# abdel-habib/mmg-clip

Measured on AMD Instinct MI355X. Metric: image-text pairs/sec (global batch), higher is better.
Workload: dtype bf16; 1 GPU; C2: train_binary_class_clf, ConvNeXt-tiny 1024x1024x1 + BERT-base S=77, LinearProjection 768->512, CLIPLoss, AdamW, all parameters trained; global_batch=256, per_gpu_batch=256, micro_batch=256, streams=text tower on a side stream, parallelism=dp1, loss_scope=local, text_dropout=HF training-mode dropout live (hidden 0.1, atte…

## Files before the change

include/mmgclip_hip.h:

```cpp
#ifndef MMGCLIP_HIP_H
#define MMGCLIP_HIP_H

#ifdef __cplusplus
extern "C" {
#endif

typedef void* mmg_stream_t;

int mmg_abi_version(void);
const char* mmg_last_error(void);
const char* mmg_target_arch(void);
int mmg_device_cu_count(void);
int mmg_set_kernel_notes(int on);
const char* mmg_last_kernel(void);
const char* mmg_gemm_plan(int op, int M, int N, int K, int cus);


int mmg_l2norm_fwd(const float* x, float* y, float* norm, int rows, int D, mmg_stream_t stream);
int mmg_l2norm_bwd(const float* y, const float* norm, const float* dy, float* dx, int rows, int D,
                   mmg_stream_t stream);

int mmg_clip_rows_fwd(const float* X, const float* Y, const float* scale, int n_loc, int N, int D, int diag_off,
                      float* lse, float* pos, float* logits, int ldl, mmg_stream_t stream);

// ... 31 lines not shown
int mmg_layernorm_bwd_f32(const void* dy, int lddy, const float* x, int ldx, const float* mean, const float* rstd,
                          const float* gamma, void* dx, int lddx, float* dgamma, float* dbeta, int M, int C,
                          const void* add, int ldadd, mmg_stream_t stream);
int mmg_layernorm_bwd(const void* dy, int lddy, const void* x, int ldx, const float* mean, const float* rstd,
                      const float* gamma, void* dx, int lddx, float* dgamma, float* dbeta, int M, int C, int patch,
                      int H, int W, const void* add, int ldadd, mmg_stream_t stream);
const char* mmg_layernorm_plan(int door, int M, int C, int res, int yf, int add);

int mmg_gelu_fwd_bf16(const void* x, void* y, long long n, mmg_stream_t stream);
int mmg_act_grad_bf16(const void* dy, const void* pre, void* out, long long n, int kind, mmg_stream_t stream);
int mmg_cast_f32_bf16(const float* x, void* y, long long n, mmg_stream_t stream);
int mmg_cast_bf16_f32(const void* x, float* y, long long n, mmg_stream_t stream);
int mmg_transpose_cast_bf16(const float* src, int R, int C, const float* rowscale, void* dst, int ldd,
                            mmg_stream_t stream);

int mmg_avgpool_fwd(const void* x, float* y, int n, int HW, int C, mmg_stream_t stream);
int mmg_avgpool_bwd(const float* dy, void* dx, int n, int HW, int C, mmg_stream_t stream);

int mmg_view_pool_fwd(const float* feat, const int* offsets, float* out, int* argmax, int S, int C, int mode, mmg_stream_t stream);
int mmg_view_pool_bwd(const float* dout, const int* offsets, const int* argmax, float* dfeat, int S, int V, int C, int mode,
                      mmg_stream_t stream);

int mmg_patchify(const float* img, void* out, int n, int Cin, int H, int W, int P, int Kp, int scale16,
                 mmg_stream_t stream);
int mmg_patchify_aug(const void* img, int src_kind, void* out, int n, int Cin, int H, int W, int P, int Kp, int scale16,
                     const int* geom, const float* tone, mmg_stream_t stream);

int mmg_adamw_step(float* p, const float* g, float* m, float* v, void* p_bf16, long long n, float lr, float beta1,
                   float beta2, float eps, float weight_decay, int step, float grad_scale, mmg_stream_t stream);


int mmg_grad_sumsq_partials(long long n);
int mmg_grad_sumsq(const float* g, long long n, double* partials, int n_partials, mmg_stream_t stream);
int mmg_grad_clip_finalize(const double* partials, int n, float max_norm, float* out, int* skipped, mmg_stream_t stream);
int mmg_adamw_step_guarded(float* p, const float* g, float* m, float* v, void* p_bf16, long long n, float lr, float beta1,
                           float beta2, float eps, float weight_decay, int step, const float* clip, const int* skipped,
                           mmg_stream_t stream);
int mmg_adamw_step_groups(float* p, const float* g, float* m, float* v, long long n, const unsigned char* chunk_group, int n_groups,
                          const float* group_lr, const float* group_wd, float beta1, float beta2, float eps, int step,
                          const float* clip, const int* skipped, mmg_stream_t stream);

int mmg_layerscale_finalize(const float* W2, const float* b2, const float* gamma, const float* dW2raw,
                            const float* db2raw, float* dW2, float* db2, float* dgamma, int C, int K,
                            mmg_stream_t stream);
int mmg_grad_relayout(const float* src, float* dst, int mode, int R, int CI, int KH, int KW, int ld_src,
                      mmg_stream_t stream);

int mmg_image_swap(void* x, const int* pairs, const int* pairs_host, int k, int n, long long rows, int C, mmg_stream_t stream);
int mmg_image_copy(const void* src, void* dst, int first, int count, int n, long long rows, int C, mmg_stream_t stream);
int mmg_scaled_add_f32(float* dst, const float* src, float alpha, long long n, mmg_stream_t stream);

int mmg_dropout_fwd(const float* x, float* y, void* keep, long long n, float p, long long seed, mmg_stream_t stream);
int mmg_dropout_bwd(const float* dy, const void* keep, float* dx, long long n, float p, mmg_stream_t stream);


int mmg_dwconv7_nhwc(const void* x, const float* w, const float* bias, const void* add, void* y, int n, int H, int W,
                     int C, int flip, mmg_stream_t stream);
int mmg_dwconv7_nhwc_mfma(const void* x, const float* w, const float* bias, const void* add, void* y, int n, int H, int W,
                          int C, int flip, mmg_stream_t stream);
int mmg_dwconv7_wgrad(const void* x, const void* dy, float* dw, float* dbias, int n, int H, int W, int C,
                      mmg_stream_t stream);


long long mmg_cnblock_packed_elems(int C, int backward);
int mmg_cnblock_pack_weights(const float* w1, const float* w2, const float* gamma, void* packed, int C, int backward,
                             mmg_stream_t stream);
int mmg_cnblock_mlp_fwd(const void* xd, const float* ln_w, const float* ln_b, float eps, const void* packed,
                        const float* b1, const float* b2, const float* gamma, const void* residual, void* y, void* hpre,
                        void* xln, void* gact, float* mean, float* rstd, int hpre_kind, long long M, int C, mmg_stream_t stream);

int mmg_cnblock_mlp_bwd_supported(int C);
int mmg_cnblock_mlp_bwd(const void* dy, const void* xd, const float* ln_w, const float* ln_b, float eps,
                        const void* packed_bwd, const float* b1, const void* hpre, void* dh, void* g, void* xln,
                        void* dxln, float* mean, float* rstd, float* ln_dw, float* ln_db, long long M, int C,
                        mmg_stream_t stream);

int mmg_cnblock_bwdw_supported(int C);
long long mmg_cnblock_bwdw_packed_elems(int C);
int mmg_cnblock_bwdw_pack(const float* w1, const float* w2, const float* ln_w, const float* ln_b, const float* layer_scale,
                          const float* b1, void* packed, float* b1f, int C, mmg_stream_t stream);
int mmg_cnblock_bwdw(const void* dy, const void* xd, const float* ln_w, const float* ln_b, float eps, const void* packed,
                     const float* b1f, void* dd, float* dW1, float* db1, float* dW2raw, float* db2raw, float* ln_dw,
                     float* ln_db, long long M, int C, mmg_stream_t stream);


int mmg_greedy_threshold_labels(const float* sim, int ld, int n, float threshold, long long* labels, int* counts, int* k_out,
                                mmg_stream_t stream);

int mmg_cluster_mean_cols_fwd(const float* logits, int ld, int n, int N, const long long* labels, const int* counts, int k,
                              float* out, int ldo, mmg_stream_t stream);
int mmg_cluster_mean_cols_bwd(const float* dout, int ldo, int n, int N, const long long* labels, const int* counts,
                              float* dlogits, int ld, mmg_stream_t stream);

int mmg_clip_labelled_rows_fwd(const float* X, const float* Y, const float* scale, const long long* row_label, int n_loc, int M,
                               int D, float* lse, float* pos, mmg_stream_t stream);
int mmg_clip_labelled_rows_bwd_row(const float* X, const float* Y, const float* scale, const float* lse_row,
                                   const long long* row_label, const float* gout, float coef, int n_loc, int M, int D,
                                   int accumulate, float* dX, float* dscale, mmg_stream_t stream);
int mmg_clip_labelled_rows_bwd_col(const float* X, const float* Y, const float* scale, const float* lse_col,
                                   const long long* col_label, const long long* row_key, int key_off, const int* counts,
                                   int n_counts, const float* gout, float coef, int n_loc, int M, int D, int accumulate,
                                   float* dX, mmg_stream_t stream);
int mmg_cluster_centroids(const float* T, const long long* labels, int N, int D, int k, float* out, mmg_stream_t stream);


int mmg_gemm_nt_fp8(const void* A, int lda, const void* B, int ldb, void* C, int ldc, int M, int N, int K,
                    const float* bias, const float* colscale, const void* residual, int ldr, void* aux_out, int ldao,
                    int epi, int out_kind, float alpha, const float* alpha_dev, mmg_stream_t stream);


int mmg_quantize_e5m2_bf16(const void* src, long long n, float* amax, void* dst, float* scales, mmg_stream_t stream);
int mmg_quantize_e5m2_bf16_delayed(const void* src, long long n, const float* amax_prev, float* amax_next, void* dst, float* scales,
                                   mmg_stream_t stream);
int mmg_quantize_e5m2_colsum_bf16(const void* src, int M, int C, const float* amax_prev, float* amax_next, void* dst, float* scales,
                                  float* colsum, mmg_stream_t stream);
int mmg_gemm_nt_fp8_bwd(const void* A, int lda, int a_e5m2, const void* B, int ldb, void* C, int ldc, int M, int N, int K,
                        const void* aux_in, int ldai, int epi, int out_kind, float alpha, const float* alpha_dev,
                        const float* alpha_dev2, mmg_stream_t stream);
int mmg_gemm_tn_fp8(const void* A, int lda, int a_e5m2, const void* B, int ldb, float* C, int ldc, int M, int N1, int N2,
                    float alpha, const float* alpha_dev, float* colsum_a, mmg_stream_t stream);

int mmg_absmax_f32(const float* src, long long n, float* amax, mmg_stream_t stream);
int mmg_quantize_e4m3_f32(const float* src, long long n, const float* amax, void* dst, float* scales, mmg_stream_t stream);

int mmg_layernorm_fwd_fp8(const void* x, int ldx, const float* gamma, const float* beta, float eps, void* y8, int ldy,
                          float* mean, float* rstd, int M, int C, mmg_stream_t stream);


int mmg_im2col_nhwc(const void* x, void* col, int n, int H, int W, int C, int KH, int KW, int stride, int pad, int Kp,
                    mmg_stream_t stream);
int mmg_col2im_nhwc(const void* dcol, void* dx, int n, int H, int W, int C, int KH, int KW, int stride, int pad, int Kp,
                    mmg_stream_t stream);
int mmg_maxpool3x3s2_nhwc(const void* x, void* y, int n, int H, int W, int C, mmg_stream_t stream);
int mmg_bn_stats_f64(const void* x, int M, int C, double* sum, double* sumsq, mmg_stream_t stream);
int mmg_bn_finalize_f64(const double* sum, const double* sumsq, int M, int C, const float* gamma, const float* beta, float eps,
                        float momentum, float* running_mean, float* running_var, int train, float* mean, float* rstd,
                        float* scale, float* shift, mmg_stream_t stream);
int mmg_bn_apply(const void* x, const float* scale, const float* shift, const void* residual, void* y, int M, int C, int relu,
                 mmg_stream_t stream);
int mmg_bn_bwd_reduce(const void* dy, const void* x, const void* out, const float* mean, const float* rstd, int M, int C,
                      float* sum_g, float* sum_gx, mmg_stream_t stream);
int mmg_bn_bwd_apply(const void* dy, const void* x, const void* out, const float* mean, const float* rstd, const float* gamma,
                     const float* sum_g, const float* sum_gx, int M, int C, void* dx, void* dres, float* dgamma, float* dbeta,
                     mmg_stream_t stream);


int mmg_attention_fwd(const void* qkv, int ld, const long long* mask, void* ctx, int ldc, float* lse, int B, int S,
                      int heads, int Hd, float scale, mmg_stream_t stream);
int mmg_attention_bwd(const void* qkv, int ld, const long long* mask, const void* ctx, int ldc, const float* lse,
                      const void* dctx, int lddc, void* dqkv, int lddq, int B, int S, int heads, int Hd, float scale,
                      mmg_stream_t stream);

int mmg_attention_long_fwd(const void* qkv, int ld, const long long* mask, void* ctx, int ldc, float* lse, int B, int S,
                           int heads, int Hd, float scale, mmg_stream_t stream);
int mmg_attention_long_bwd(const void* qkv, int ld, const long long* mask, const void* ctx, int ldc, const float* lse,
                           const void* dctx, int lddc, void* dqkv, int lddq, float* delta_ws, int B, int S, int heads,
                           int Hd, float scale, mmg_stream_t stream);

int mmg_attention_varlen_fwd(const void* qkv, int ld, const int* cu_seqlens, void* ctx, int ldc, float* lse, int B, int S_max,
                             int heads, int Hd, float scale, mmg_stream_t stream);
int mmg_attention_varlen_bwd(const void* qkv, int ld, const int* cu_seqlens, const void* ctx, int ldc, const float* lse,
                             const void* dctx, int lddc, void* dqkv, int lddq, int B, int S_max, int heads, int Hd,
                             float scale, mmg_stream_t stream);

int mmg_attention_dropout_fwd(const void* qkv, int ld, const long long* mask, const int* cu_seqlens, void* ctx, int ldc,
                              float* lse, int B, int S, int heads, int Hd, float scale, float p, unsigned long long seed,
// ... 35 lines not shown
```

mmg-clip_amd/mmgclip/kernels.py:

```python
import ctypes
import os

import torch

from . import _hip
from ._hip import call, ptr, stream
from .profile import PROFILE

BF16 = torch.bfloat16


def layernorm_fwd(x, gamma, beta, eps, patch_hw=None, want_stats=True):
    M, C = x.shape
    if patch_hw is None:
        y = torch.empty(M, C, device=x.device, dtype=BF16)
        patch, H, W = 0, 0, 0
    else:
        H, W = patch_hw
        y = torch.empty((M // (H * W)) * (H // 2) * (W // 2), 4 * C, device=x.device, dtype=BF16)
        patch = 1
    mean = torch.empty(M, device=x.device, dtype=torch.float32) if want_stats else None
    rstd = torch.empty(M, device=x.device, dtype=torch.float32) if want_stats else None
    PROFILE.timed("layernorm_fwd_kernel", 8.0 * M * C, 4 * M * C,
                  lambda: call("mmg_layernorm_fwd", ptr(x), x.stride(0), ptr(gamma), ptr(beta), float(eps), ptr(y), y.stride(0), ptr(mean),
# ... 117 lines not shown

def avgpool_bwd(dy, n, HW, C, out=None):
    dx = out if out is not None else torch.empty(n * HW, C, device=dy.device, dtype=BF16)
    call("mmg_avgpool_bwd", ptr(dy), ptr(dx), n, HW, C, stream())
    return dx


def _images(x, n):
    assert x.dtype == BF16 and x.dim() == 2 and x.is_contiguous() and n > 0 and x.shape[0] % n == 0, "bf16 [n * rows, C], contiguous"
    _hip.require_gpu(x)
    return x.shape[0] // n, x.shape[1]


def image_swap_(x, n, pairs_dev, pairs_host, k, offset=0):
    rows, C = _images(x, n)
    if k:
        assert pairs_dev.dtype == torch.int32 and pairs_dev.is_contiguous() and 2 * (offset + k) <= pairs_dev.numel() == len(pairs_host)
    call("mmg_image_swap", ptr(x), ctypes.c_void_p(pairs_dev.data_ptr() + 8 * offset) if k else None,
         ctypes.c_void_p(ctypes.addressof(pairs_host) + 8 * offset) if k else None, k, n, rows, C, stream())
    return x


def image_copy(src, dst, n, first, count):
    rows, C = _images(src, n)
    assert dst.shape == src.shape and dst.dtype == BF16 and dst.is_contiguous()
    _hip.require_gpu(dst)
    call("mmg_image_copy", ptr(src), ptr(dst), first, count, n, rows, C, stream())
    return dst


def scaled_add_(dst, src, alpha):
    assert dst.dtype == src.dtype == torch.float32 and dst.is_contiguous() and src.is_contiguous() and dst.numel() == src.numel()
    _hip.require_gpu(dst, src)
    call("mmg_scaled_add_f32", ptr(dst), ptr(src), float(alpha), dst.numel(), stream())
    return dst


def view_pool_fwd(feat, offsets, S, mode, out=None, argmax=None):
    V, C = feat.shape
    assert feat.dtype == torch.float32 and feat.is_contiguous() and offsets.dtype == torch.int32 and offsets.numel() == S + 1
    _hip.require_gpu(feat, offsets)
    y = out if out is not None else torch.empty(S, C, device=feat.device, dtype=torch.float32)
    if mode == 1 and argmax is None:
        argmax = torch.empty(S, C, device=feat.device, dtype=torch.int32)
    call("mmg_view_pool_fwd", ptr(feat), ptr(offsets), ptr(y), ptr(argmax) if mode == 1 else None, S, C, mode, stream())
    return y, (argmax if mode == 1 else None)


def view_pool_bwd(dout, offsets, argmax, V, mode, out=None):
    S, C = dout.shape
    assert dout.dtype == torch.float32 and dout.is_contiguous() and offsets.dtype == torch.int32 and offsets.numel() == S + 1
    _hip.require_gpu(dout, offsets)
    dx = out if out is not None else torch.empty(V, C, device=dout.device, dtype=torch.float32)
    call("mmg_view_pool_bwd", ptr(dout), ptr(offsets), ptr(argmax), ptr(dx), S, V, C, mode, stream())
    return dx


PIXEL_KINDS = {torch.float32: 0, torch.uint16: 1, torch.uint8: 2}


def stack_images(images):
    if images[0].dtype == torch.uint16:
        return torch.stack([t.view(torch.int16) for t in images]).view(torch.uint16)
    return torch.stack(list(images))


def patchify(img, P, Kp, scale16, geom=None, tone=None):
    n, Cin, H, W = img.shape
    if img.dtype not in PIXEL_KINDS:
        raise TypeError(f"pixels must be float32 in [0, 1], uint16 or uint8, got {img.dtype}")
    assert img.is_contiguous(), "pixels must be contiguous [n, Cin, H, W]"
    _hip.require_gpu(img, geom, tone)
    out = torch.empty(n * (H // P) * (W // P), Kp, device=img.device, dtype=BF16)
    if img.dtype == torch.float32 and geom is None and tone is None:
        call("mmg_patchify", ptr(img), ptr(out), n, Cin, H, W, P, Kp, 1 if scale16 else 0, stream())
        return out
    assert geom is None or (geom.dtype == torch.int32 and geom.is_contiguous() and tuple(geom.shape) == (n, 4)), "geom: int32 [n, 4]"
    assert tone is None or (tone.dtype == torch.float32 and tone.is_contiguous() and tuple(tone.shape) == (n, 2)), "tone: fp32 [n, 2]"
    call("mmg_patchify_aug", ptr(img), PIXEL_KINDS[img.dtype], ptr(out), n, Cin, H, W, P, Kp, 1 if scale16 else 0, ptr(geom), ptr(tone),
         stream())
    return out


def adamw_step(p, g, m, v, p16, lr, beta1, beta2, eps, wd, step, grad_scale=1.0):
    call("mmg_adamw_step", ptr(p), ptr(g), ptr(m), ptr(v), ptr(p16), p.numel(), float(lr), float(beta1), float(beta2),
         float(eps), float(wd), int(step), float(grad_scale), stream())


def grad_sumsq_partials(n):
    return int(_hip.load().mmg_grad_sumsq_partials(int(n)))


def grad_sumsq(g, partials, offset=0, count=None):
    assert g.dtype == torch.float32 and g.is_contiguous() and partials.dtype == torch.float64 and partials.is_contiguous()
    _hip.require_gpu(g, partials)
    count = grad_sumsq_partials(g.numel()) if count is None else int(count)
    assert 0 <= offset and offset + count <= partials.numel()
    call("mmg_grad_sumsq", ptr(g), g.numel(), ptr(partials[offset:]) if count else ptr(partials), count, stream())


def grad_clip_finalize(partials, n, max_norm, out, skipped=None):
    assert partials.dtype == torch.float64 and out.dtype == torch.float32 and out.numel() >= 3 and n <= partials.numel()
    assert skipped is None or (skipped.dtype == torch.int32 and skipped.numel() >= 1)
    _hip.require_gpu(partials, out, skipped)
    call("mmg_grad_clip_finalize", ptr(partials), int(n), 0.0 if max_norm is None else float(max_norm), ptr(out), ptr(skipped), stream())


def adamw_step_guarded(p, g, m, v, p16, lr, beta1, beta2, eps, wd, step, clip, skipped=None):
    assert clip.dtype == torch.float32 and clip.numel() >= 3 and (skipped is None or skipped.dtype == torch.int32)
    call("mmg_adamw_step_guarded", ptr(p), ptr(g), ptr(m), ptr(v), ptr(p16), p.numel(), float(lr), float(beta1), float(beta2),
         float(eps), float(wd), int(step), ptr(clip), ptr(skipped), stream())


ADAMW_MAX_GROUPS = 128


def adamw_step_groups(p, g, m, v, chunk_group, group_lr, group_wd, beta1, beta2, eps, step, clip=None, skipped=None):
    n_groups = len(group_lr)
    assert len(group_wd) == n_groups and chunk_group.dtype == torch.uint8 and chunk_group.is_contiguous()
    assert chunk_group.numel() * 64 == p.numel() == g.numel() == m.numel() == v.numel()
    assert clip is None or (clip.dtype == torch.float32 and clip.numel() >= 3)
    assert skipped is None or skipped.dtype == torch.int32
    _hip.require_gpu(p, g, m, v, chunk_group, clip, skipped)
    lrs = (ctypes.c_float * max(n_groups, 1))(*[float(x) for x in group_lr])
    wds = (ctypes.c_float * max(n_groups, 1))(*[float(x) for x in group_wd])
    call("mmg_adamw_step_groups", ptr(p), ptr(g), ptr(m), ptr(v), p.numel(), ptr(chunk_group), n_groups, lrs, wds, float(beta1),
         float(beta2), float(eps), int(step), ptr(clip), ptr(skipped), stream())


def dwconv_mfma_pays(n, H, W, C, flip):
    return H * W >= 96 * 96 and C <= 256


def dwconv7(x, w49, bias, n, H, W, C, add=None, flip=False, out=None):
    y = out if out is not None else torch.empty(n * H * W, C, device=x.device, dtype=BF16)
    px = n * H * W * C
    mode = os.environ.get("MMG_DWCONV_MFMA", "auto")
    if mode == "1" or (mode == "auto" and dwconv_mfma_pays(n, H, W, C, flip)):
        PROFILE.timed("dwconv7_mfma_kernel", 98.0 * px, (6 if add is not None else 4) * px,
                      lambda: call("mmg_dwconv7_nhwc_mfma", ptr(x), ptr(w49), ptr(bias), ptr(add), ptr(y), n, H, W, C, 1 if flip else 0, stream()),
                      f"n={n} {H}x{W} C={C}" + (" +add" if add is not None else ""))
        return y
    fam = "dwconv7_rows2_kernel" if os.environ.get("MMG_DWCONV_ROWS2", "1") != "0" else "dwconv7_kernel"
    PROFILE.timed(fam, 98.0 * px, (6 if add is not None else 4) * px,
                  lambda: call("mmg_dwconv7_nhwc", ptr(x), ptr(w49), ptr(bias), ptr(add), ptr(y), n, H, W, C, 1 if flip else 0, stream()),
                  f"n={n} {H}x{W} C={C}" + (" +add" if add is not None else ""))
    return y


def dwconv7_wgrad(x, dy, dw49, dbias, n, H, W, C):
    px = n * H * W * C
    fam = "dwconv7_wgrad_rows2_kernel" if os.environ.get("MMG_DWCONV_ROWS2", "1") != "0" else "dwconv7_wgrad_kernel"
    PROFILE.timed(fam, 98.0 * px, 4 * px,
                  lambda: call("mmg_dwconv7_wgrad", ptr(x), ptr(dy), ptr(dw49), ptr(dbias), n, H, W, C, stream()), f"n={n} {H}x{W} C={C}")


def cnblock_supported(C):
    return C in (96, 128, 192, 256, 384, 512)


def cnblock_pack(w1, w2, gamma=None, backward=False):
    C = w1.shape[1]
    backward = int(backward)
    n = _hip.load().mmg_cnblock_packed_elems(C, backward)
    if n <= 0:
        raise ValueError(f"fused CNBlock MLP: C={C} is not supported")
# ... 225 lines not shown
```

mmg-clip_amd/mmgclip/networks/convnext.py:

```python
import ctypes
import os

import torch
import torch.nn as nn

from .. import _hip
from .. import kernels as K
from .. import linalg as L
from .._hip import call, ptr, stream
from ..params import backward_finished, last_backward
from . import convnext_sd as SD
from .convnext_plan import BlockSaved, Knobs, decide_saves, fused_forward, plan_block, saving_form
from .tower import Tower, as_pixels, augment_tables, backward_parts, conv_weight_rows, fold_conv_grad, forward_parts

CONFIGS = {
    "tiny": dict(depths=(3, 3, 9, 3), dims=(96, 192, 384, 768)),
    "small": dict(depths=(3, 3, 27, 3), dims=(96, 192, 384, 768)),
    "base": dict(depths=(3, 3, 27, 3), dims=(128, 256, 512, 1024)),
}
LN_EPS = 1e-6


def _fused_save_maxc():
    return int(os.environ.get("MMG_MLP_FUSED_SAVE_MAXC", "384"))
# ... 110 lines not shown
                w1, w2, gamma = blk.block[3].weight.data, blk.block[5].weight.data, blk.layer_scale.data.reshape(C)
                if scales is not None and scales[b] != 1.0:
                    gamma = gamma * scales[b]
                wc[key + ".gamma"] = gamma
                b += 1
                wc[key + ".w49"] = blk.block[0].weight.data.reshape(C, 49).t().contiguous()
                wc[key + ".w1"] = K.cast_bf16(w1)
                wc[key + ".w1t"] = K.transpose_cast_bf16(w1)
                wc[key + ".w2"] = K.cast_bf16(w2)
                wc[key + ".w2gt"] = K.transpose_cast_bf16(w2, gamma)
                if p.kind == "fp8":
                    wc[key + ".w1f8"], wc[key + ".s1"] = K.quantize_e4m3(w1)
                    wc[key + ".w2f8"], wc[key + ".s2"] = K.quantize_e4m3(w2)
                    if p.fp8_bwd_weights:
                        wc[key + ".w2gt8"], wc[key + ".s2gt"] = K.quantize_e4m3((w2 * gamma.reshape(C, 1)).t().contiguous())
                        wc[key + ".w1t8"], wc[key + ".s1t"] = K.quantize_e4m3(w1.t().contiguous())
                elif p.kind == "fused":
                    wc[key + ".mlp"] = K.cnblock_pack(w1, w2)
                    if p.fused_bwd:
                        wc[key + ".mlpb"] = K.cnblock_pack(w1, w2, gamma, backward=p.fused_bwd)
                    if p.bwdw:
                        wc[key + ".bwdw"] = K.cnblock_bwdw_pack(w1, w2, blk.block[2].weight.data, blk.block[2].bias.data, gamma,
                                                                blk.block[3].bias.data)
            if si < 3:
                wds = conv_weight_rows(f[2 + 2 * si][1].weight.data)
                wc[f"ds{si}.w"] = K.cast_bf16(wds)
                wc[f"ds{si}.wt"] = K.transpose_cast_bf16(wds)
        return wc

    def _decide_saves(self, n_alive, H, W, device, ckpt=False, more=()):
        return decide_saves(self.plan or self._plan_blocks(), self.depths, ((n_alive, H, W),) + tuple(more),
                            torch.cuda.get_device_properties(device).total_memory, ckpt, self.save_ln_mode, self.save_gelu_mode,
                            self.fp8_bwd_mode if self.fp8 else "0")

    def _saving(self, p, dec, M):
        return saving_form(p, dec, M, self.save_dgelu) if dec is not None else (None, None, False, False)

    def _fwd_fused(self, x, d, blk, key, p, dec, out=None):
        bwd, aux_kind, keep_ln, keep_g = self._saving(p, dec, d.shape[0])
        keep = aux_kind is not None
        outs = K.cnblock_mlp_fwd(d, blk.block[2].weight.data, blk.block[2].bias.data, LN_EPS, self._wc[key + ".mlp"],
                                 blk.block[3].bias.data, blk.block[5].bias.data, self._wc[key + ".gamma"], x,
                                 want_hpre=keep, want_stats=keep, want_xln=keep_ln, want_gact=keep_g, hpre_kind=1 if aux_kind == "dgelu" else 0,
                                 out=out)
        xn, hpre, mean, rstd = outs[:4]
        if dec is None:
            return xn, None
        return xn, BlockSaved(x, d, mean, rstd, hpre, aux_kind, outs[4] if keep_ln else None, outs[-1] if keep_g else None, bwd)

    def _fwd_gemm(self, x, d, blk, key, p, dec, out=None):
        C, wc, save = p.C, self._wc, dec is not None
        bwd, aux_kind, keep_ln, keep_g = self._saving(p, dec, d.shape[0])
        hpre = torch.empty(x.shape[0], 4 * C, device=x.device, dtype=torch.bfloat16) if save else None
        epi = L.EPI_GELU_DAUX if aux_kind == "dgelu" else L.EPI_GELU
        if p.kind == "fp8":
            ln, mean, rstd = K.layernorm_fwd_fp8(d, blk.block[2].weight.data, blk.block[2].bias.data, LN_EPS, want_stats=save)
            g = L.gemm_nt_fp8(ln, wc[key + ".w1f8"], bias=blk.block[3].bias.data, aux_out=hpre, epi=epi, out_kind=L.OUT_E4M3,
                              alpha_dev=wc[key + ".s1"][1:])
            xn = L.gemm_nt_fp8(g, wc[key + ".w2f8"], out=out, bias=blk.block[5].bias.data, colscale=wc[key + ".gamma"],
                               residual=x, alpha_dev=wc[key + ".s2"][1:])
        else:
            ln, mean, rstd = K.layernorm_fwd(d, blk.block[2].weight.data, blk.block[2].bias.data, LN_EPS, want_stats=save)
            g = L.gemm_nt(ln, wc[key + ".w1"], bias=blk.block[3].bias.data, aux_out=hpre, epi=epi)
            xn = L.gemm_nt(g, wc[key + ".w2"], out=out, bias=blk.block[5].bias.data, colscale=wc[key + ".gamma"], residual=x)
        if not save:
            return xn, None
        return xn, BlockSaved(x, d, mean, rstd, hpre, aux_kind, ln if keep_ln else None, g if keep_g else None, bwd)

    def _forward_mb(self, img, plan, dec, sched=None, tabs=None):
        f, wc = self.model.features, self._wc
        save = dec is not None
        n, _, H, W = img.shape
        h, w_ = H // 4, W // 4
        saved = {"maps": [(h, w_)]}
        steps = table = None
        if sched is not None:
            steps = sched.steps
            if sched.table:
                host = (ctypes.c_int * len(sched.table))(*sched.table)
                table = (torch.tensor(sched.table, dtype=torch.int32, device=img.device), host)
            saved["sd"] = (steps, table)
        b = 0
        p0 = K.patchify(img, 4, self.kp, self.scale16, *(tabs or (None, None)))
        s0 = L.gemm_nt(p0, wc["stem.w"], bias=f[0][0].bias.data)
        x, mean, rstd = K.layernorm_fwd(s0, f[0][1].weight.data, f[0][1].bias.data, LN_EPS, want_stats=save)
        if save:
            saved["stem"] = (p0, s0, mean, rstd)
        for si, p in enumerate(plan):
            mlp = self._fwd_fused if fused_forward(p, save) else self._fwd_gemm
            for bi, blk in enumerate(f[1 + 2 * si]):
                key = f"{si}.{bi}"
                step = steps[b] if steps is not None else None
                b += 1
                if step is None or step.n_k == n:
                    d = K.dwconv7(x, wc[key + ".w49"], blk.block[0].bias.data, n, h, w_, p.C)
                    x, rec = mlp(x, d, blk, key, p, dec)
                elif step.n_k == 0:
                    rec = None
                else:
                    K.image_swap_(x, n, *(table or (None, None)), len(step.pairs), step.offset)
                    n_k, Mk = step.n_k, step.n_k * h * w_
                    xk, out = x[:Mk], torch.empty_like(x)
                    d = K.dwconv7(xk, wc[key + ".w49"], blk.block[0].bias.data, n_k, h, w_, p.C)
                    _, rec = mlp(xk, d, blk, key, p, dec, out=out[:Mk])
                    K.image_copy(x, out, n, n_k, n - n_k)
                    x = out
                if save:
                    saved[key] = rec
            if si < 3:
                lnm = f[2 + 2 * si][0]
                ld, mean, rstd = K.layernorm_fwd(x, lnm.weight.data, lnm.bias.data, LN_EPS, patch_hw=(h, w_), want_stats=save)
                xn = L.gemm_nt(ld, wc[f"ds{si}.w"], bias=f[2 + 2 * si][1].bias.data)
                if save:
                    saved[f"ds{si}"] = (x, mean, rstd, ld)
                x = xn
                h, w_ = h // 2, w_ // 2
                saved["maps"].append((h, w_))
        feat = K.avgpool_fwd(x, n, h * w_, self.dims[-1])
        saved["shape"] = (n, H, W)
        return feat, saved

    def _ln_bwd(self, dln, d, mean, rstd, blk):
        return K.layernorm_bwd(dln, d, mean, rstd, blk.block[2].weight.data, self._g(blk.block[2], "weight"), self._g(blk.block[2], "bias"))

    def _bwd_bwdw(self, dx, rec, blk, key, tmp):
        packed, b1f = self._wc[key + ".bwdw"]
        return K.cnblock_bwdw(dx, rec.d, blk.block[2].weight.data, blk.block[2].bias.data, LN_EPS, packed, b1f,
                              self._g(blk.block[3], "weight"), self._g(blk.block[3], "bias"), tmp[key + ".dw2raw"], tmp[key + ".db2raw"],
                              self._g(blk.block[2], "weight"), self._g(blk.block[2], "bias"))

    def _bwd_fused(self, dx, rec, blk, key, tmp):
        fuse_ln = rec.d.shape[1] <= 128
        dh, g, ln, dln, mean, rstd = K.cnblock_mlp_bwd(
            dx, rec.d, blk.block[2].weight.data, blk.block[2].bias.data, LN_EPS, self._wc[key + ".mlpb"], blk.block[3].bias.data, rec.aux,
            ln_grads=(self._g(blk.block[2], "weight"), self._g(blk.block[2], "bias")) if fuse_ln else None)
        L.gemm_tn_acc(dx, g, tmp[key + ".dw2raw"], colsum=tmp[key + ".db2raw"])
        del g
        L.gemm_tn_acc(dh, ln, self._g(blk.block[3], "weight"), colsum=self._g(blk.block[3], "bias"))
        del ln, dh
        return dln if fuse_ln else self._ln_bwd(dln, rec.d, mean, rstd, blk)

    def _bwd_fp8(self, dx, rec, blk, key, tmp):
        wc = self._wc
        dy8, sdy = K.quantize_e5m2(dx, self._e5m2_state.setdefault(key, {}) if self.fp8_delayed else None, colsum=tmp[key + ".db2raw"])
        dh8 = L.gemm_nt_fp8_bwd(dy8, wc[key + ".w2gt8"], aux_in=rec.aux, epi=L.EPI_MUL_AUX, out_kind=L.OUT_E5M2,
                                alpha_dev=wc[key + ".s2gt"][1:])
        L.gemm_tn_fp8_acc(dy8, rec.g, tmp[key + ".dw2raw"], alpha_dev=sdy[1:])
        L.gemm_tn_fp8_acc(dh8, rec.ln, self._g(blk.block[3], "weight"), alpha_dev=sdy[1:], colsum=self._g(blk.block[3], "bias"))
        dln = L.gemm_nt_fp8_bwd(dh8, wc[key + ".w1t8"], alpha_dev=wc[key + ".s1t"][1:], alpha_dev2=sdy[1:])
        del dh8, dy8
        return self._ln_bwd(dln, rec.d, rec.mean, rec.rstd, blk)

    def _bwd_gemm(self, dx, rec, blk, key, tmp):
        wc = self._wc
        if rec.g is not None:
            g = rec.g
            dh = L.gemm_nt(dx, wc[key + ".w2gt"], epi=L.EPI_MUL_AUX if rec.aux_kind == "dgelu" else L.EPI_DGELU_ONLY, aux_in=rec.aux)
        else:
            g = torch.empty_like(rec.aux)
            dh = L.gemm_nt(dx, wc[key + ".w2gt"], epi=L.EPI_DGELU, aux_in=rec.aux, aux_out=g)
        L.gemm_tn_acc(dx, g, tmp[key + ".dw2raw"], colsum=tmp[key + ".db2raw"])
        del g
        ln = rec.ln if rec.ln is not None else \
            K.layernorm_fwd(rec.d, blk.block[2].weight.data, blk.block[2].bias.data, LN_EPS, want_stats=False)[0]
        L.gemm_tn_acc(dh, ln, self._g(blk.block[3], "weight"), colsum=self._g(blk.block[3], "bias"))
        del ln
        dln = L.gemm_nt(dh, wc[key + ".w1t"])
        del dh
        return self._ln_bwd(dln, rec.d, rec.mean, rec.rstd, blk)

    def _backward_mb(self, dfeat, saved, tmp, final=False, announce=False):
        f, wc, A = self.model.features, self._wc, self._arena
        n, H, W = saved["shape"]
        maps = saved["maps"]
        steps, table = saved.get("sd", (None, None))
        b = sum(self.depths)
        h, w_ = maps[3]
        dx = K.avgpool_bwd(dfeat, n, h * w_, self.dims[-1])
        for si in range(3, -1, -1):
            C = self.dims[si]
            if si < 3:
                x, mean, rstd, ld = saved[f"ds{si}"]
                conv, lnm = f[2 + 2 * si][1], f[2 + 2 * si][0]
                L.gemm_tn_acc(dx, ld, tmp[f"ds{si}.dw"], colsum=self._g(conv, "bias"))
                dld = L.gemm_nt(dx, wc[f"ds{si}.wt"])
                h, w_ = maps[si]
                dx = K.layernorm_bwd(dld, x, mean, rstd, lnm.weight.data, self._g(lnm, "weight"), self._g(lnm, "bias"),
                                     patch_hw=(h, w_))
                del dld
            for bi in range(self.depths[si] - 1, -1, -1):
                blk = f[1 + 2 * si][bi]
                key = f"{si}.{bi}"
                rec = saved[key]
                b -= 1
                step = steps[b] if steps is not None else None
                if step is None or step.n_k == n:
                    dd = getattr(self, "_bwd_" + rec.bwd)(dx, rec, blk, key, tmp)
                    K.dwconv7_wgrad(rec.x, dd, tmp[key + ".dw49"], self._g(blk.block[0], "bias"), n, h, w_, C)
                    dx = K.dwconv7(dd, wc[key + ".w49"], None, n, h, w_, C, add=dx, flip=True)
                    del dd
                elif step.n_k:
                    n_k, Mk = step.n_k, step.n_k * h * w_
                    dxk, dxn = dx[:Mk], torch.empty_like(dx)
                    dd = getattr(self, "_bwd_" + rec.bwd)(dxk, rec, blk, key, tmp)
                    K.dwconv7_wgrad(rec.x, dd, tmp[key + ".dw49"], self._g(blk.block[0], "bias"), n_k, h, w_, C)
                    K.dwconv7(dd, wc[key + ".w49"], None, n_k, h, w_, C, add=dxk, flip=True, out=dxn[:Mk])
                    del dd, dxk
                    K.image_copy(dx, dxn, n, n_k, n - n_k)
                    dx = K.image_swap_(dxn, n, *(table or (None, None)), len(step.pairs), step.offset)
            if final:
                self._finalize_stage(tmp, si)
                if announce:
                    A.mark_ready((f"features.{1 + 2 * si}.",) + ((f"features.{2 + 2 * si}.",) if si < 3 else ()))
        p0, s0, mean, rstd = saved["stem"]
        ds0 = K.layernorm_bwd(dx, s0, mean, rstd, f[0][1].weight.data, self._g(f[0][1], "weight"), self._g(f[0][1], "bias"))
        L.gemm_tn_acc(ds0, p0, tmp["stem.dw"], colsum=self._g(f[0][0], "bias"))
        if final:
            fold_conv_grad(tmp["stem.dw"], self._g(f[0][0], "weight"), self.dims[0], self.in_chans, 4, 4)

    def _alloc_tmp(self, device):
        z = lambda *s: torch.zeros(*s, device=device, dtype=torch.float32)
        tmp = {"stem.dw": z(self.dims[0], self.kp)}
        for si in range(4):
            C = self.dims[si]
            for bi in range(self.depths[si]):
                key = f"{si}.{bi}"
                tmp[key + ".dw2raw"], tmp[key + ".db2raw"], tmp[key + ".dw49"] = z(C, 4 * C), z(C), z(49, C)
            if si < 3:
                tmp[f"ds{si}.dw"] = z(self.dims[si + 1], 4 * C)
        return tmp

    def _finalize_stage(self, tmp, si):
        f = self.model.features
        C = self.dims[si]
        scales = self._wc["sd.scales"]
        for bi, blk in enumerate(f[1 + 2 * si]):
            key = f"{si}.{bi}"
            s = scales[sum(self.depths[:si]) + bi] if scales is not None else 1.0
            dgamma = self._g(blk, "layer_scale") if s == 1.0 else torch.zeros(C, device=tmp[key + ".dw2raw"].device, dtype=torch.float32)
            call("mmg_layerscale_finalize", ptr(blk.block[5].weight.data), ptr(blk.block[5].bias.data),
                 ptr(self._wc[key + ".gamma"]), ptr(tmp[key + ".dw2raw"]), ptr(tmp[key + ".db2raw"]),
                 ptr(self._g(blk.block[5], "weight")), ptr(self._g(blk.block[5], "bias")),
                 ptr(dgamma), C, 4 * C, stream())
            if s != 1.0:
                K.scaled_add_(self._g(blk, "layer_scale"), dgamma, s)
            call("mmg_grad_relayout", ptr(tmp[key + ".dw49"]), ptr(self._g(blk.block[0], "weight")), 1, C, 1, 7, 7, C,
                 stream())
        if si < 3:
            fold_conv_grad(tmp[f"ds{si}.dw"], self._g(f[2 + 2 * si][1], "weight"), self.dims[si + 1], C, 2, 2)

    def feature_map_shape(self, H, W):
        h, w = H // 4, W // 4
        for _ in range(3):
            h, w = h // 2, w // 2
        return h, w

    def forward(self, images, sample_ids=None):
        plan = None
        if isinstance(images, (list, tuple)):
            if not images or any(not torch.is_tensor(t) or t.dim() != 3 for t in images):
                raise ValueError("a list of images must hold [Cin, H, W] tensors")
            for t in images:
                _hip.require_gpu(t)
                if t.shape[-2] < 32 or t.shape[-1] < 32:
                    raise ValueError(f"ConvNeXt needs at least 32x32 pixels, got {tuple(t.shape)}")
            plan = group_by_size([tuple(t.shape[-2:]) for t in images], self.micro_batch)
            device = images[0].device
        else:
            _hip.require_gpu(images)
            if images.shape[-2] < 32 or images.shape[-1] < 32:
                raise ValueError(f"ConvNeXt needs at least 32x32 pixels, got {tuple(images.shape)}")
            device = images.device
        anchor = self._record_forward(device)
        seed = None
        if self.stochastic_depth_active():
            if self.next_drop_seed is not None:
                seed, self.next_drop_seed = int(self.next_drop_seed), None
            else:
                seed = self._drop_seeds.draw()
            ids = list(range(len(images))) if sample_ids is None else [int(i) for i in sample_ids]
            if len(ids) != len(images):
                raise ValueError(f"sample_ids names {len(ids)} images, the input holds {len(images)}")
            seed = (seed, ids)
        aug = self._draw_augment(len(images), sample_ids)
        if plan is None:
            return _ConvNextFn.apply(self, as_pixels(images).contiguous(), anchor, None, seed, aug)
        return _ConvNextFn.apply(self, [as_pixels(t) for t in images], anchor, plan, seed, aug)


def group_by_size(sizes, micro_batch):
    if micro_batch < 1:
        raise ValueError(f"micro_batch must be positive, got {micro_batch}")
    groups = {}
    for i, hw in enumerate(sizes):
        groups.setdefault(tuple(int(v) for v in hw), []).append(i)
    mbs = [idx[k:k + micro_batch] for idx in groups.values() for k in range(0, len(idx), micro_batch)]
    inverse = [0] * len(sizes)
    for pos, i in enumerate(j for mb in mbs for j in mb):
        inverse[i] = pos
# ... 71 lines not shown
```

Measured before the change: 838.6 image-text pairs/sec.

## Fuse ConvNeXt stem GEMM with LayerNorm in forward and backward kernels

Adds HIP kernels that fuse the stem patch-projection GEMM with its LayerNorm. In the forward pass this avoids writing the pre-norm activation s0. In the backward pass the kernel recomputes s0 from the patches, then does the LayerNorm backward and the weight-gradient GEMM in one pass with LDS reductions and atomics. This removes the s0 round-trip through memory, an intermediate ds0 tensor, and several kernel launches, all on the largest-resolution activation (1024x1024 input, stride 4). The cost is a recomputed GEMM in backward and atomic reductions of dW, both enabled by default through an environment flag.

```diff
diff --git a/include/mmgclip_hip.h b/include/mmgclip_hip.h
--- a/include/mmgclip_hip.h
+++ b/include/mmgclip_hip.h
@@ -137,6 +137,13 @@
 int mmg_cnblock_bwdw(const void* dy, const void* xd, const float* ln_w, const float* ln_b, float eps, const void* packed,
                      const float* b1f, void* dd, float* dW1, float* db1, float* dW2raw, float* db2raw, float* ln_dw,
                      float* ln_db, long long M, int C, mmg_stream_t stream);
+
+int mmg_stem_supported(int C, int kp);
+int mmg_stem_fwd(const void* p0, const void* w, const float* bias, const float* ln_w, const float* ln_b, float eps, void* x,
+                 float* mean, float* rstd, long long M, int C, int kp, mmg_stream_t stream);
+int mmg_stem_bwd(const void* dx, const void* p0, const void* w, const float* bias, const float* ln_w, const float* mean,
+                 const float* rstd, float* dW, float* db, float* ln_dw, float* ln_db, long long M, int C, int kp,
+                 mmg_stream_t stream);
 
 
 int mmg_greedy_threshold_labels(const float* sim, int ld, int n, float threshold, long long* labels, int* counts, int* k_out,
diff --git a/mmg-clip_amd/csrc/stem.hip b/mmg-clip_amd/csrc/stem.hip
--- /dev/null
+++ b/mmg-clip_amd/csrc/stem.hip
@@ -0,0 +1,324 @@
+#include "common.h"
+
+typedef __attribute__((ext_vector_type(4))) unsigned st_u32x4;
+typedef __attribute__((address_space(3))) bf16x4 st_lds_v4;
+
+template <int C, int KP> struct StemCfg {
+    static_assert((C == 96 || C == 128) && (KP == 32 || KP == 64), "stem: C in {96, 128}, kp in {32, 64}");
+    static constexpr int CT = C / 16;
+    static constexpr int KS = KP / 32;
+    static constexpr int NT = KP / 16;
+    static constexpr int WAVES = 4;
+    static constexpr int PP = KP * 2 + 32;
+    static constexpr int DP = C * 2 + 32;
+    static constexpr int RB = 32;
+    static constexpr int P0IMG = RB * PP, DXIMG = RB * DP, STIMG = 2 * RB * 4, WAVE_LDS = P0IMG + DXIMG + STIMG;
+    static constexpr int WIMG = CT * KS * 1024;
+    static constexpr int OFF_IMG = WIMG;
+    static constexpr int RED = (C * KP + 3 * C) * 4;
+    static constexpr int LDS = OFF_IMG + WAVES * WAVE_LDS;
+    static_assert(RED <= WAVES * WAVE_LDS, "the reduction buffer aliases the row images");
+    static_assert(LDS <= 80 * 1024, "two workgroups per CU");
+    static constexpr int BWD_WPS = C * KP <= 96 * 32 ? 2 : 1;
+};
+
+struct StemFwdArgs {
+    const bf16_t* p0; const bf16_t* w; const float* bias; const float* ln_w; const float* ln_b; float eps;
+    bf16_t* x; float* mean; float* rstd; long long M; int nt;
+};
+
+struct StemBwdArgs {
+    const bf16_t* dx; const bf16_t* p0; const bf16_t* w; const float* bias; const float* ln_w; const float* mean; const float* rstd;
+    float* dW; float* db; float* ln_dw; float* ln_db; long long M;
+};
+
+__device__ __forceinline__ float st_sum16(float v) {
+    v += __int_as_float(__builtin_amdgcn_mov_dpp(__float_as_int(v), 0xB1, 0xf, 0xf, true));
+    v += __int_as_float(__builtin_amdgcn_mov_dpp(__float_as_int(v), 0x4E, 0xf, 0xf, true));
+    v += __int_as_float(__builtin_amdgcn_mov_dpp(__float_as_int(v), 0x141, 0xf, 0xf, true));
+    v += __int_as_float(__builtin_amdgcn_mov_dpp(__float_as_int(v), 0x140, 0xf, 0xf, true));
+    return v;
+}
+__device__ __forceinline__ float st_sum_lg(float v) {
+    v += __shfl_xor(v, 16, 64); v += __shfl_xor(v, 32, 64);
+    return v;
+}
+__device__ __forceinline__ bf16x4 st_tr(const char* p) { return __builtin_amdgcn_ds_read_tr16_b64_v4i16((st_lds_v4*)p); }
+
+template <int C, int KP, int WPS>
+__global__ __launch_bounds__(256, WPS) void stem_fwd_kernel(const StemFwdArgs a) {
+    typedef StemCfg<C, KP> Cfg;
+    constexpr int CT = Cfg::CT, KS = Cfg::KS, G = 4;
+    const int lane = threadIdx.x & 63, wave = threadIdx.x >> 6;
+    const int li = lane & 15, lg = lane >> 4;
+    const bool odd = (lg & 1) != 0;
+
+    __shared__ __attribute__((aligned(16))) float s_gb[2 * C];
+    for (int i = threadIdx.x; i < C; i += 256) { s_gb[i] = a.ln_w[i]; s_gb[C + i] = a.ln_b[i]; }
+    __syncthreads();
+    bf16x8 wf[CT][KS];
+    f32x4 bia[CT];
+#pragma unroll
+    for (int ct = 0; ct < CT; ++ct) {
+#pragma unroll
+        for (int ks = 0; ks < KS; ++ks) wf[ct][ks] = *reinterpret_cast<const bf16x8*>(a.w + (size_t)(16 * ct + li) * KP + 32 * ks + 8 * lg);
+        bia[ct] = *reinterpret_cast<const f32x4*>(a.bias + 16 * ct + 4 * lg);
+    }
+    const float inv_c = 1.0f / (float)C;
+    const long long ntiles = (a.M + 63) / 64;
+    for (long long t = (long long)blockIdx.x * Cfg::WAVES + wave; t < ntiles; t += (long long)gridDim.x * Cfg::WAVES) {
+        const long long r0 = t * 64;
+        bf16x8 pf[G][KS];
+#pragma unroll
+        for (int g = 0; g < G; ++g) {
+            const long long row = r0 + 16 * g + li, rc = row < a.M ? row : a.M - 1;
+#pragma unroll
+            for (int ks = 0; ks < KS; ++ks) pf[g][ks] = *reinterpret_cast<const bf16x8*>(a.p0 + (size_t)rc * KP + 32 * ks + 8 * lg);
+        }
+#pragma unroll
+        for (int g = 0; g < G; ++g) {
+            const long long row = r0 + 16 * g + li;
+            const bool live = row < a.M;
+            f32x4 acc[CT];
+#pragma unroll
+            for (int ct = 0; ct < CT; ++ct) {
+                acc[ct] = bia[ct];
+#pragma unroll
+                for (int ks = 0; ks < KS; ++ks) acc[ct] = __builtin_amdgcn_mfma_f32_16x16x32_bf16(wf[ct][ks], pf[g][ks], acc[ct], 0, 0, 0);
+            }
+            float s = 0.f;
+#pragma unroll
+            for (int ct = 0; ct < CT; ++ct)
+#pragma unroll
+                for (int e = 0; e < 4; ++e) { acc[ct][e] = bf2f(f2bf(acc[ct][e])); s += acc[ct][e]; }
+            const float mu = st_sum_lg(s) * inv_c;
+            float q = 0.f;
+#pragma unroll
+            for (int ct = 0; ct < CT; ++ct)
+#pragma unroll
+                for (int e = 0; e < 4; ++e) { acc[ct][e] -= mu; q += acc[ct][e] * acc[ct][e]; }
+            const float rs = rsqrtf(st_sum_lg(q) * inv_c + a.eps);
+            unsigned pk[CT][2];
+#pragma unroll
+            for (int ct = 0; ct < CT; ++ct) {
+                const f32x4 gam = *reinterpret_cast<const f32x4*>(s_gb + 16 * ct + 4 * lg), bet = *reinterpret_cast<const f32x4*>(s_gb + C + 16 * ct + 4 * lg);
+                float o[4];
+#pragma unroll
+                for (int e = 0; e < 4; ++e) o[e] = acc[ct][e] * rs * gam[e] + bet[e];
+                pk[ct][0] = pack2bf(o[0], o[1]); pk[ct][1] = pack2bf(o[2], o[3]);
+            }
+            bf16_t* xrow = a.x + (size_t)(live ? row : 0) * C;
+#pragma unroll
+            for (int c = 0; c < CT / 2; ++c) {
+                const unsigned s0 = odd ? pk[2 * c][0] : pk[2 * c + 1][0], s1 = odd ? pk[2 * c][1] : pk[2 * c + 1][1];
+                const unsigned r0_ = __shfl_xor(s0, 16, 64), r1_ = __shfl_xor(s1, 16, 64);
+                const uint4 v = odd ? make_uint4(r0_, r1_, pk[2 * c + 1][0], pk[2 * c + 1][1]) : make_uint4(pk[2 * c][0], pk[2 * c][1], r0_, r1_);
+                const int ch = odd ? 32 * c + 16 + 4 * (lg - 1) : 32 * c + 4 * lg;
+                if (live) store16_stream(xrow + ch, v, a.nt != 0);
+            }
+            if (live && lg == 0) {
+                if (a.mean) a.mean[row] = mu;
+                if (a.rstd) a.rstd[row] = rs;
+            }
+            __builtin_amdgcn_sched_barrier(0);
+        }
+    }
+}
+
+template <int C, int KP>
+__global__ __launch_bounds__(256, (StemCfg<C, KP>::BWD_WPS)) void stem_bwd_kernel(const StemBwdArgs a) {
+    typedef StemCfg<C, KP> Cfg;
+    constexpr int CT = Cfg::CT, KS = Cfg::KS, NT = Cfg::NT, PP = Cfg::PP, DP = Cfg::DP, RB = Cfg::RB;
+    extern __shared__ __attribute__((aligned(16))) char smem[];
+    const int tid = threadIdx.x, lane = tid & 63, wave = tid >> 6;
+    const int li = lane & 15, lg = lane >> 4, q = (lane >> 2) & 3, p = lane & 3;
+
+    for (int i = tid; i < CT * KS * 64; i += 256) {
+        const int l = i & 63, ks = (i >> 6) % KS, ct = (i >> 6) / KS;
+        *reinterpret_cast<uint4*>(smem + i * 16) = *reinterpret_cast<const uint4*>(a.w + (size_t)(16 * ct + (l & 15)) * KP + 32 * ks + 8 * (l >> 4));
+    }
+    float gam[CT], bia[CT];
+#pragma unroll
+    for (int ct = 0; ct < CT; ++ct) { gam[ct] = a.ln_w[16 * ct + li]; bia[ct] = a.bias[16 * ct + li]; }
+    __syncthreads();
+
+    char* pimg = smem + Cfg::OFF_IMG + wave * Cfg::WAVE_LDS;
+    char* dimg = pimg + Cfg::P0IMG;
+    float* simg = reinterpret_cast<float*>(dimg + Cfg::DXIMG);
+    const int p_wr = li * PP + lg * 16;
+    const int tr_p = (4 * lg + q) * PP + 8 * p;
+    const int tr_d = (4 * lg + q) * DP + 8 * p;
+
+    f32x4 dwacc[CT][NT];
+    float dg[CT], dbt[CT], dbs[CT];
+#pragma unroll
+    for (int ct = 0; ct < CT; ++ct) {
+        dg[ct] = 0.f; dbt[ct] = 0.f; dbs[ct] = 0.f;
+#pragma unroll
+        for (int nt = 0; nt < NT; ++nt) dwacc[ct][nt] = f32x4{0.f, 0.f, 0.f, 0.f};
+    }
+    const float inv_c = 1.0f / (float)C;
+    const long long nsteps = (a.M + RB - 1) / RB;
+    for (long long st = (long long)blockIdx.x * Cfg::WAVES + wave; st < nsteps; st += (long long)gridDim.x * Cfg::WAVES) {
+        const long long r0 = st * RB;
+        bf16x8 pa[2][KS];
+#pragma unroll
+        for (int t2 = 0; t2 < 2; ++t2) {
+            const long long row = r0 + 16 * t2 + li, rc = row < a.M ? row : a.M - 1;
+#pragma unroll
+            for (int ks = 0; ks < KS; ++ks) pa[t2][ks] = *reinterpret_cast<const bf16x8*>(a.p0 + (size_t)rc * KP + 32 * ks + 8 * lg);
+        }
+        uint4 dxr[CT];
+        int d_wr[CT];
+#pragma unroll
+        for (int n = 0; n < CT; ++n) {
+            const int byte = (lane + 64 * n) * 16, r = byte / (2 * C), cb = byte % (2 * C);
+            const long long row = r0 + r;
+            const bool live = row < a.M;
+            const uint4 v = *reinterpret_cast<const uint4*>(a.dx + (size_t)(live ? row : a.M - 1) * C + cb / 2);
+            dxr[n] = live ? v : make_uint4(0u, 0u, 0u, 0u);
+            d_wr[n] = r * DP + cb;
+        }
+        float stat;
+        {
+            const long long row = r0 + (lane & 31), rc = row < a.M ? row : a.M - 1;
+            stat = lane < 32 ? a.mean[rc] : a.rstd[rc];
+        }
+        asm volatile("" ::: "memory");
+#pragma unroll
+        for (int t2 = 0; t2 < 2; ++t2)
+#pragma unroll
+            for (int ks = 0; ks < KS; ++ks) *reinterpret_cast<bf16x8*>(pimg + p_wr + t2 * 16 * PP + ks * 64) = pa[t2][ks];
+#pragma unroll
+        for (int n = 0; n < CT; ++n) *reinterpret_cast<uint4*>(dimg + d_wr[n]) = dxr[n];
+        simg[lane] = stat;
+        asm volatile("s_waitcnt lgkmcnt(0)" ::: "memory");
+
+        unsigned dsu[CT][4];
+#pragma unroll
+        for (int t2 = 0; t2 < 2; ++t2) {
+            float xh[CT][4];
+            bf16x4 dq[CT];
+            const f32x4 mu = *reinterpret_cast<const f32x4*>(simg + 16 * t2 + 4 * lg), rs = *reinterpret_cast<const f32x4*>(simg + RB + 16 * t2 + 4 * lg);
+            float s1[4] = {0.f, 0.f, 0.f, 0.f}, s2[4] = {0.f, 0.f, 0.f, 0.f};
+#pragma unroll
+            for (int ct = 0; ct < CT; ++ct) {
+                f32x4 acc = f32x4{0.f, 0.f, 0.f, 0.f};
+#pragma unroll
+                for (int ks = 0; ks < KS; ++ks)
+                    acc = __builtin_amdgcn_mfma_f32_16x16x32_bf16(pa[t2][ks], *reinterpret_cast<const bf16x8*>(smem + ((ct * KS + ks) * 64 + lane) * 16), acc, 0, 0, 0);
+                dq[ct] = st_tr(dimg + tr_d + t2 * 16 * DP + ct * 32);
+#pragma unroll
+                for (int e = 0; e < 4; ++e) {
+                    const float s0 = bf2f(f2bf(acc[e] + bia[ct]));
+                    const float x = (s0 - mu[e]) * rs[e], dv = bf2f((bf16_t)dq[ct][e]), g = dv * gam[ct];
+                    xh[ct][e] = x;
+                    s1[e] += g;
+                    s2[e] += g * x;
+                    dg[ct] += dv * x;
+                    dbt[ct] += dv;
+                }
+            }
+#pragma unroll
+            for (int e = 0; e < 4; ++e) { s1[e] = st_sum16(s1[e]) * inv_c; s2[e] = st_sum16(s2[e]) * inv_c; }
+#pragma unroll
+            for (int ct = 0; ct < CT; ++ct) {
+                float o[4];
+#pragma unroll
+                for (int e = 0; e < 4; ++e) {
+                    o[e] = rs[e] * (bf2f((bf16_t)dq[ct][e]) * gam[ct] - s1[e] - xh[ct][e] * s2[e]);
+                    dbs[ct] += bf2f(f2bf(o[e]));
+                }
+                dsu[ct][2 * t2] = pack2bf(o[0], o[1]); dsu[ct][2 * t2 + 1] = pack2bf(o[2], o[3]);
+            }
+        }
+        bf16x8 pt[NT];
+#pragma unroll
+        for (int nt = 0; nt < NT; ++nt) {
+            const bf16x4 lo = st_tr(pimg + tr_p + nt * 32), hi = st_tr(pimg + tr_p + 16 * PP + nt * 32);
+            pt[nt] = bf16x8{lo[0], lo[1], lo[2], lo[3], hi[0], hi[1], hi[2], hi[3]};
+        }
+#pragma unroll
+        for (int ct = 0; ct < CT; ++ct) {
+            const bf16x8 df = __builtin_bit_cast(bf16x8, (st_u32x4{dsu[ct][0], dsu[ct][1], dsu[ct][2], dsu[ct][3]}));
+#pragma unroll
+            for (int nt = 0; nt < NT; ++nt) dwacc[ct][nt] = __builtin_amdgcn_mfma_f32_16x16x32_bf16(df, pt[nt], dwacc[ct][nt], 0, 0, 0);
+        }
+    }
+
+    float* red = reinterpret_cast<float*>(smem + Cfg::OFF_IMG);
+    __syncthreads();
+    for (int i = tid; i < C * KP + 3 * C; i += 256) red[i] = 0.f;
+    __syncthreads();
+#pragma unroll
+    for (int ct = 0; ct < CT; ++ct) {
+#pragma unroll
+        for (int nt = 0; nt < NT; ++nt)
+#pragma unroll
+            for (int e = 0; e < 4; ++e) atomicAdd(&red[(16 * ct + 4 * lg + e) * KP + 16 * nt + li], dwacc[ct][nt][e]);
+        const float g = st_sum_lg(dg[ct]), b = st_sum_lg(dbt[ct]), s = st_sum_lg(dbs[ct]);
+        if (lg == 0) {
+            atomicAdd(&red[C * KP + 16 * ct + li], g);
+            atomicAdd(&red[C * KP + C + 16 * ct + li], b);
+            atomicAdd(&red[C * KP + 2 * C + 16 * ct + li], s);
+        }
+    }
+    __syncthreads();
+    for (int i = tid; i < C * KP; i += 256) atomicAdd(a.dW + i, red[i]);
+    for (int i = tid; i < C; i += 256) {
+        atomicAdd(a.ln_dw + i, red[C * KP + i]);
+        atomicAdd(a.ln_db + i, red[C * KP + C + i]);
+        atomicAdd(a.db + i, red[C * KP + 2 * C + i]);
+    }
+}
+
+MMG_API int mmg_stem_supported(int C, int kp) { return (C == 96 || C == 128) && (kp == 32 || kp == 64) ? 1 : 0; }
+
+template <int C, int KP, int WPS>
+static void stem_fwd_launch(const StemFwdArgs& a, hipStream_t stream) {
+    const long long wg_tiles = (a.M + 255) / 256;
+    const long long cap = (long long)mmg_cu_count_cached() * WPS;
+    hipLaunchKernelGGL((stem_fwd_kernel<C, KP, WPS>), dim3((unsigned)(wg_tiles < cap ? wg_tiles : cap)), dim3(256), 0, stream, a);
+}
+
+template <int C, int KP>
+static void stem_bwd_launch(const StemBwdArgs& a, hipStream_t stream) {
+    typedef StemCfg<C, KP> Cfg;
+    const long long wg_steps = (a.M + 4 * Cfg::RB - 1) / (4 * Cfg::RB);
+    const long long cap = (long long)mmg_cu_count_cached() * Cfg::BWD_WPS;
+    mmg_allow_lds(stem_bwd_kernel<C, KP>, Cfg::LDS);
+    hipLaunchKernelGGL((stem_bwd_kernel<C, KP>), dim3((unsigned)(wg_steps < cap ? wg_steps : cap)), dim3(256), Cfg::LDS, stream, a);
+}
+
+MMG_API int mmg_stem_fwd(const void* p0, const void* w, const float* bias, const float* ln_w, const float* ln_b, float eps, void* x,
+                         float* mean, float* rstd, long long M, int C, int kp, hipStream_t stream) {
+    MMG_CHECK_ARG(mmg_stem_supported(C, kp), "mmg_stem_fwd: C=%d kp=%d is not supported (C in {96, 128}, kp in {32, 64})", C, kp);
+    MMG_CHECK_ARG(M > 0, "mmg_stem_fwd: M=%lld must be positive", M);
+    MMG_CHECK_ARG(p0 && w && bias && ln_w && ln_b && x, "mmg_stem_fwd: null pointer");
+    MMG_CHECK_ARG((mean == nullptr) == (rstd == nullptr), "mmg_stem_fwd: mean and rstd are saved together (both or neither)");
+    StemFwdArgs a{(const bf16_t*)p0, (const bf16_t*)w, bias, ln_w, ln_b, eps, (bf16_t*)x, mean, rstd, M,
+                  M * C * 2 >= (256LL << 20) ? 1 : 0};
+    MMG_NOTE_KERNEL("stem_fwd_kernel<%d, %d, %d>", C, kp, C == 96 && kp == 32 ? 3 : 2);
+    if (C == 96 && kp == 32) stem_fwd_launch<96, 32, 3>(a, stream);
+    else if (C == 96) stem_fwd_launch<96, 64, 2>(a, stream);
+    else if (kp == 32) stem_fwd_launch<128, 32, 2>(a, stream);
+    else stem_fwd_launch<128, 64, 2>(a, stream);
+    MMG_LAUNCH_CHECK("mmg_stem_fwd");
+    return 0;
+}
+
+MMG_API int mmg_stem_bwd(const void* dx, const void* p0, const void* w, const float* bias, const float* ln_w, const float* mean,
+                         const float* rstd, float* dW, float* db, float* ln_dw, float* ln_db, long long M, int C, int kp,
+                         hipStream_t stream) {
+    MMG_CHECK_ARG(mmg_stem_supported(C, kp), "mmg_stem_bwd: C=%d kp=%d is not supported (C in {96, 128}, kp in {32, 64})", C, kp);
+    MMG_CHECK_ARG(M > 0, "mmg_stem_bwd: M=%lld must be positive", M);
+    MMG_CHECK_ARG(dx && p0 && w && bias && ln_w && mean && rstd && dW && db && ln_dw && ln_db, "mmg_stem_bwd: null pointer");
+    StemBwdArgs a{(const bf16_t*)dx, (const bf16_t*)p0, (const bf16_t*)w, bias, ln_w, mean, rstd, dW, db, ln_dw, ln_db, M};
+    MMG_NOTE_KERNEL("stem_bwd_kernel<%d, %d>", C, kp);
+    if (C == 96 && kp == 32) stem_bwd_launch<96, 32>(a, stream);
+    else if (C == 96) stem_bwd_launch<96, 64>(a, stream);
+    else if (kp == 32) stem_bwd_launch<128, 32>(a, stream);
+    else stem_bwd_launch<128, 64>(a, stream);
+    MMG_LAUNCH_CHECK("mmg_stem_bwd");
+    return 0;
+}
diff --git a/mmg-clip_amd/mmgclip/kernels.py b/mmg-clip_amd/mmgclip/kernels.py
--- a/mmg-clip_amd/mmgclip/kernels.py
+++ b/mmg-clip_amd/mmgclip/kernels.py
@@ -223,6 +223,41 @@
     return out
 
 
+def stem_supported(C, kp):
+    return bool(_hip.load().mmg_stem_supported(int(C), int(kp)))
+
+
+def stem_fused_enabled():
+    return os.environ.get("MMG_STEM_FUSED", "1") != "0"
+
+
+def stem_fwd(p0, w, bias, ln_w, ln_b, eps, want_stats=True):
+    M, kp = p0.shape
+    C = w.shape[0]
+    assert p0.dtype == BF16 and w.dtype == BF16 and p0.is_contiguous() and w.is_contiguous() and w.shape[1] == kp
+    _hip.require_gpu(p0, w, bias, ln_w, ln_b)
+    x = torch.empty(M, C, device=p0.device, dtype=BF16)
+    mean = torch.empty(M, device=p0.device, dtype=torch.float32) if want_stats else None
+    rstd = torch.empty(M, device=p0.device, dtype=torch.float32) if want_stats else None
+    PROFILE.timed("stem_fwd_kernel", 2.0 * M * C * kp, 2 * M * (kp + C) + (8 * M if want_stats else 0) + 2 * C * kp,
+                  lambda: call("mmg_stem_fwd", ptr(p0), ptr(w), ptr(bias), ptr(ln_w), ptr(ln_b), float(eps), ptr(x), ptr(mean), ptr(rstd),
+                               M, C, kp, stream()), f"M={M} C={C} kp={kp}" + (" +stats" if want_stats else ""))
+    return x, mean, rstd
+
+
+def stem_bwd(dx, p0, w, bias, ln_w, mean, rstd, dW, db, ln_dw, ln_db):
+    M, kp = p0.shape
+    C = w.shape[0]
+    assert dx.dtype == BF16 and p0.dtype == BF16 and dx.is_contiguous() and p0.is_contiguous() and tuple(dx.shape) == (M, C)
+    assert mean.dtype == rstd.dtype == torch.float32 and mean.numel() == rstd.numel() == M
+    for t, n in ((dW, C * kp), (db, C), (ln_dw, C), (ln_db, C)):
+        assert t.dtype == torch.float32 and t.is_contiguous() and t.numel() == n
+    _hip.require_gpu(dx, p0, w, bias, ln_w, mean, rstd, dW, db, ln_dw, ln_db)
+    PROFILE.timed("stem_bwd_kernel", 2.0 * M * C * kp, 2 * M * (kp + C) + 8 * M + 6 * C * kp,
+                  lambda: call("mmg_stem_bwd", ptr(dx), ptr(p0), ptr(w), ptr(bias), ptr(ln_w), ptr(mean), ptr(rstd), ptr(dW), ptr(db),
+                               ptr(ln_dw), ptr(ln_db), M, C, kp, stream()), f"M={M} C={C} kp={kp}")
+
+
 def adamw_step(p, g, m, v, p16, lr, beta1, beta2, eps, wd, step, grad_scale=1.0):
     call("mmg_adamw_step", ptr(p), ptr(g), ptr(m), ptr(v), ptr(p16), p.numel(), float(lr), float(beta1), float(beta2),
          float(eps), float(wd), int(step), float(grad_scale), stream())
diff --git a/mmg-clip_amd/mmgclip/networks/convnext.py b/mmg-clip_amd/mmgclip/networks/convnext.py
--- a/mmg-clip_amd/mmgclip/networks/convnext.py
+++ b/mmg-clip_amd/mmgclip/networks/convnext.py
@@ -216,8 +216,12 @@
             saved["sd"] = (steps, table)
         b = 0
         p0 = K.patchify(img, 4, self.kp, self.scale16, *(tabs or (None, None)))
-        s0 = L.gemm_nt(p0, wc["stem.w"], bias=f[0][0].bias.data)
-        x, mean, rstd = K.layernorm_fwd(s0, f[0][1].weight.data, f[0][1].bias.data, LN_EPS, want_stats=save)
+        if K.stem_fused_enabled() and K.stem_supported(self.dims[0], self.kp):
+            s0 = None
+            x, mean, rstd = K.stem_fwd(p0, wc["stem.w"], f[0][0].bias.data, f[0][1].weight.data, f[0][1].bias.data, LN_EPS, want_stats=save)
+        else:
+            s0 = L.gemm_nt(p0, wc["stem.w"], bias=f[0][0].bias.data)
+            x, mean, rstd = K.layernorm_fwd(s0, f[0][1].weight.data, f[0][1].bias.data, LN_EPS, want_stats=save)
         if save:
             saved["stem"] = (p0, s0, mean, rstd)
         for si, p in enumerate(plan):
@@ -347,8 +351,12 @@
                 if announce:
                     A.mark_ready((f"features.{1 + 2 * si}.",) + ((f"features.{2 + 2 * si}.",) if si < 3 else ()))
         p0, s0, mean, rstd = saved["stem"]
-        ds0 = K.layernorm_bwd(dx, s0, mean, rstd, f[0][1].weight.data, self._g(f[0][1], "weight"), self._g(f[0][1], "bias"))
-        L.gemm_tn_acc(ds0, p0, tmp["stem.dw"], colsum=self._g(f[0][0], "bias"))
+        if s0 is None:
+            K.stem_bwd(dx, p0, wc["stem.w"], f[0][0].bias.data, f[0][1].weight.data, mean, rstd, tmp["stem.dw"], self._g(f[0][0], "bias"),
+                       self._g(f[0][1], "weight"), self._g(f[0][1], "bias"))
+        else:
+            ds0 = K.layernorm_bwd(dx, s0, mean, rstd, f[0][1].weight.data, self._g(f[0][1], "weight"), self._g(f[0][1], "bias"))
+            L.gemm_tn_acc(ds0, p0, tmp["stem.dw"], colsum=self._g(f[0][0], "bias"))
         if final:
             fold_conv_grad(tmp["stem.dw"], self._g(f[0][0], "weight"), self.dims[0], self.in_chans, 4, 4)
 
```

New measurement: 847.8 image-text pairs/sec (median of 6 runs). 1.01x the previous value.
